# ElesionKyrie/Extreme-Video-Compression-With-Prediction-Using-Pre-trainded-Diffusion-Models-

Measured on AMD Instinct MI355X. Metric: decoded frames/sec (128x128x30) at q3, higher is better.
Workload: dtype f32

## Files before the change

extreme-video-compression-with-prediction-using-pre-trainded-diffusion-models-_amd/csrc/conv_igemm.hip:

```cpp
#include <hip/hip_runtime.h>
#include <stdint.h>
#include <stdio.h>
#include "../../include/evc_hip.h"

typedef float f32x16 __attribute__((ext_vector_type(16)));
typedef __attribute__((address_space(3))) void lds_void;
typedef const __attribute__((address_space(1))) void glb_void;

#ifndef EVC_CONV_TAIL
#define EVC_CONV_TAIL 1
#endif
#ifndef EVC_CONV_TM1
#define EVC_CONV_TM1 1
#endif
#ifndef EVC_SPLIT_WIDE_TILES
#define EVC_SPLIT_WIDE_TILES 1
#endif

#ifndef EVC_SPLIT_INTERLEAVE
#define EVC_SPLIT_INTERLEAVE 5
#endif

namespace {

// ... 1019 lines not shown
            __builtin_amdgcn_sched_barrier(0);
            asm volatile("s_waitcnt vmcnt(2) lgkmcnt(0)\n\ts_barrier" ::: "memory");
            __builtin_amdgcn_sched_barrier(0);
            wb ^= 1; ++sidx;
        }
        {
            EVC_RR_NEXT_W()
            EVC_RR_FRAGS(1)
            EVC_RR_TERMS(0, SP::NTERM)
            __syncthreads();
            wb ^= 1; ++sidx;
        }
        {
            EVC_RR_NEXT_W()
            __builtin_amdgcn_sched_barrier(0);
            EVC_RR_FRAGS(2)
            EVC_RR_TERMS(0, SP::NTERM / 2)
            __builtin_amdgcn_sched_barrier(0);
            store_a(ab ^ 1);
            __builtin_amdgcn_sched_barrier(0);
            EVC_RR_TERMS(SP::NTERM / 2, SP::NTERM)
            __builtin_amdgcn_sched_barrier(0);
            __syncthreads();
            wb ^= 1; ++sidx;
        }
    }
#undef EVC_RR_TERMS
#undef EVC_RR_FRAGS
#undef EVC_RR_NEXT_W

    conv_epilogue<TM, TN, WM>(p, acc, m0, n0, split, wm, wn, l31, half, tail);
}

template <bool PARTIAL, bool RES, bool STATS, bool ACT>
__device__ __forceinline__ void wide_epilogue_t(const ConvK& p, f32x16 (&acc)[4][3], char* lds, int m0, int n0, int split,
                                                int wave, int lane, bool tail) {
    constexpr int TM = 4, TN = 3, BM = 256, RS = 36;
    const int wm = wave >> 1, wn = wave & 1;
    const int l31 = lane & 31, half = lane >> 5;
    const int ws_m0 = tail ? p.tail_first * BM : 0;
    const size_t ws_M = tail ? (size_t)p.tail_rows : (size_t)p.M;
    const float ascale = p.w_hdr[0] / in_scale(p);
    const float oscale = p.out_scale;
    const bool has_res = RES && (!ACT || p.res != nullptr), has_stats = STATS && (!ACT || p.stats != nullptr);
    float* const patch0 = reinterpret_cast<float*>(lds) + wave * 2 * 32 * RS;
    const int wr = lane >> 3, wc = (lane & 7) * 4;
    const int mw = m0 + wm * 32 * TM;
    const int prow = 4 * half * RS + l31;
    constexpr int RD = 4;
    float4 rq[RD][4];
    const auto res_load = [&](int t, float4 (&dst)[4]) {
        const int jj = t / TM, ii = t - jj * TM;
        const float* rp = p.res + (size_t)(mw + ii * 32 + wr) * p.ld_res + n0 + wn * 32 * TN + jj * 32 + wc;
#pragma unroll
        for (int k = 0; k < 4; ++k) dst[k] = *reinterpret_cast<const float4*>(rp + (size_t)(8 * k) * p.ld_res);
    };
    if (has_res) {
#pragma unroll
        for (int t = 0; t < RD - 1; ++t) res_load(t, rq[t]);
    }
#pragma unroll
    for (int j = 0; j < TN; ++j) {
        const int cj = n0 + wn * 32 * TN + j * 32;
        const float bias = (!PARTIAL && p.bias) ? p.bias[cj + l31] : 0.f;
        float4 ssum = make_float4(0.f, 0.f, 0.f, 0.f), ssq = make_float4(0.f, 0.f, 0.f, 0.f);
#pragma unroll
        for (int i = 0; i < TM; ++i) {
            const int mb = mw + i * 32;
            const int tt = j * TM + i;
            if (has_res && tt + RD - 1 < TM * TN) res_load(tt + RD - 1, rq[(tt + RD - 1) % RD]);
            float* const P = patch0 + ((i * TN + j) & 1) * 32 * RS;
#pragma unroll
            for (int r = 0; r < 16; ++r) P[prow + ((r & 3) + 8 * (r >> 2)) * RS] = acc[i][j][r] * ascale + bias;
#pragma unroll
            for (int k = 0; k < 4; ++k) {
                float4 q = *reinterpret_cast<const float4*>(P + (wr + 8 * k) * RS + wc);
                const int m = mb + wr + 8 * k;
                if (!PARTIAL) {
                    if (has_res) { const float4& rr = rq[tt % RD][k]; q.x += rr.x; q.y += rr.y; q.z += rr.z; q.w += rr.w; }
                    q.x *= oscale; q.y *= oscale; q.z *= oscale; q.w *= oscale;
                    if (ACT) { q.x = act_fn(q.x, p.act_out); q.y = act_fn(q.y, p.act_out); q.z = act_fn(q.z, p.act_out); q.w = act_fn(q.w, p.act_out); }
                    if (STATS) {
                        ssum.x += q.x; ssum.y += q.y; ssum.z += q.z; ssum.w += q.w;
                        ssq.x += q.x * q.x; ssq.y += q.y * q.y; ssq.z += q.z * q.z; ssq.w += q.w * q.w;
                    }
                }
                float* dst = PARTIAL ? p.ws + ((size_t)split * ws_M + (m - ws_m0)) * p.Co + cj + wc
                                     : p.out + (size_t)m * p.ld_out + cj + wc;
                *reinterpret_cast<float4*>(dst) = q;
            }
            if (has_stats && (i & 1)) {
#pragma unroll
                for (int d = 8; d <= 32; d <<= 1) {
                    ssum.x += __shfl_xor(ssum.x, d); ssum.y += __shfl_xor(ssum.y, d); ssum.z += __shfl_xor(ssum.z, d); ssum.w += __shfl_xor(ssum.w, d);
                    ssq.x += __shfl_xor(ssq.x, d); ssq.y += __shfl_xor(ssq.y, d); ssq.z += __shfl_xor(ssq.z, d); ssq.w += __shfl_xor(ssq.w, d);
                }
                if (wr == 0) {
                    float* sp = p.stats + ((size_t)(m0 / 64 + wm * 2 + (i >> 1)) * p.Co + cj + wc) * 2;
                    *reinterpret_cast<float4*>(sp) = make_float4(ssum.x, ssq.x, ssum.y, ssq.y);
                    *reinterpret_cast<float4*>(sp + 4) = make_float4(ssum.z, ssq.z, ssum.w, ssq.w);
                }
                ssum = make_float4(0.f, 0.f, 0.f, 0.f); ssq = make_float4(0.f, 0.f, 0.f, 0.f);
            }
        }
    }
}

__device__ __forceinline__ void wide_epilogue(const ConvK& p, f32x16 (&acc)[4][3], char* lds, int m0, int n0, int split,
                                              int wave, int lane, bool tail) {
    const bool partial = p.splits > 1 || tail;
    if (partial) wide_epilogue_t<true, false, false, false>(p, acc, lds, m0, n0, split, wave, lane, tail);
    else if (p.act_out != EVC_ACT_NONE) wide_epilogue_t<false, true, true, true>(p, acc, lds, m0, n0, split, wave, lane, tail);
    else if (p.res && p.stats) wide_epilogue_t<false, true, true, false>(p, acc, lds, m0, n0, split, wave, lane, tail);
    else if (p.stats) wide_epilogue_t<false, false, true, false>(p, acc, lds, m0, n0, split, wave, lane, tail);
    else if (p.res) wide_epilogue_t<false, true, false, false>(p, acc, lds, m0, n0, split, wave, lane, tail);
    else wide_epilogue_t<false, false, false, false>(p, acc, lds, m0, n0, split, wave, lane, tail);
}

#ifndef EVC_WIDE_VMEM_EVERY
#define EVC_WIDE_VMEM_EVERY 36
#endif
#ifndef EVC_WIDE_BDIST
#define EVC_WIDE_BDIST 1
#endif
#ifndef EVC_WIDE_BUFFER_LOADS
#define EVC_WIDE_BUFFER_LOADS 0
#endif
#ifndef EVC_WIDE_ABL
#define EVC_WIDE_ABL 0
#endif
#ifdef EVC_WIDE_STAMPS
__device__ unsigned long long g_wide_stamps[8192 * 8];
#define EVC_STAMP(k) if (threadIdx.x == 0) g_wide_stamps[(blockIdx.x & 8191) * 8 + (k)] = __builtin_readcyclecounter();
#else
#define EVC_STAMP(k)
#endif
template <int MODE, int NU, bool X2>
__global__ __launch_bounds__(256, 1) void conv_wide_kernel(ConvK p) {
    typedef Split<2> SP;
    typedef f16x8 vec;
    constexpr int TM = 4, TN = 3, BM = 256, BN = 192, RB = 32;
    constexpr bool HAS_COEF = MODE == MODE_AFFINE || MODE == MODE_AFFINE_SILU;
    extern __shared__ __attribute__((aligned(16))) char smem_b[];
    const int W = p.W, SW = W + 2;
    const int R = BM / W;
    const int SPX = (R + 2) * SW;
    const int APL = SPX * RB;
    const int HPL = SPX * 16;
    char* const As = smem_b;

    const int tid = threadIdx.x;
    const int lane = tid & 63;
    const int wave = __builtin_amdgcn_readfirstlane(tid >> 6);
    const int wm = wave >> 1, wn = wave & 1;
    const int l31 = lane & 31, half = lane >> 5;

#ifdef EVC_WIDE_STAGGER_TEST
    if (blockIdx.x < 256) for (int q = 0; q < (int)((blockIdx.x >> 3) & 3) * EVC_WIDE_STAGGER_TEST; ++q) __builtin_amdgcn_s_sleep(127);
#endif
    EVC_STAMP(0)
    const bool tail = (int)blockIdx.x >= p.tail_first;
    const int tq = tail ? ((int)blockIdx.x - p.tail_first) / p.tail_splits : 0;
    const int m0 = (tail ? p.tail_first + tq : (int)blockIdx.x) * BM;
    const int n0 = blockIdx.y * BN;
    const int split = tail ? (int)blockIdx.x - p.tail_first - tq * p.tail_splits : (int)blockIdx.z;
    const int sps = tail ? p.tail_sps : p.steps_per_split;
    const int c_begin = p.cut_chunk ? (split ? p.cut_chunk : 0) : min(p.nchunk, split * (sps / 9));
    const int c_end = p.cut_chunk ? (split ? p.nchunk : p.cut_chunk) : min(p.nchunk, c_begin + sps / 9);

    const int bimg = m0 / p.HW;
    const int y0 = (m0 - bimg * p.HW) / W;
    const int Ct = p.C0 + p.C1;

    const int kh = tid & 1;
    unsigned goff0[NU], goff1[NU];
    int slds[NU];
    bool sval[NU], sex[NU];
#pragma unroll
    for (int k = 0; k < NU; ++k) {
        int pp = (tid + 256 * k) >> 1;
        if (pp >= (R + 2) * W) pp = tid >> 1;
        const int sr = pp / W, x = pp - sr * W;
        sex[k] = true;
        const int y = y0 + sr - 1;
        sval[k] = sex[k] && y >= 0 && y < p.H;
        const unsigned pix = (unsigned)((bimg * p.H + (sval[k] ? y : 0)) * W + x);
        goff0[k] = (pix * (unsigned)p.ld0 + 8u * kh) * 4u;
        goff1[k] = (pix * (unsigned)p.ld1 + 8u * kh) * 4u;
        const int spx = (sex[k] ? sr : 0) * SW + x + 1;
        slds[k] = kh * HPL + spx * 16;
    }
    int abase[TM];
#pragma unroll
    for (int i = 0; i < TM; ++i) {
        const int ml = wm * 128 + i * 32 + l31;
        const int r = ml / W, x = ml - r * W;
        abase[i] = half * HPL + (r * SW + x) * 16;
    }
    const auto tap_off = [&](int t) { return ((t / 3) * SW + (t % 3)) * 16; };
    const unsigned planeB = (unsigned)p.CoPad * RB;
    const unsigned slab = 2u * planeB;
    const unsigned w_tap = (unsigned)p.nchunk * slab;
    const unsigned wlane = (unsigned)(n0 + wn * 96 + l31) * RB + 16u * (unsigned)(half ^ ((l31 >> 3) & 1));
    const char* const wbase = reinterpret_cast<const char*>(p.w);
#if EVC_WIDE_BUFFER_LOADS
    typedef int i32x4 __attribute__((ext_vector_type(4)));
    const __amdgpu_buffer_rsrc_t wrsrc = __builtin_amdgcn_make_buffer_rsrc(const_cast<char*>(wbase), 0, 0x7fffffff, 0x00020000);
    auto load_b = [&](vec (&bb)[TN][2], int c, int t) {
        const int so = (int)((unsigned)t * w_tap + (unsigned)c * slab);
#pragma unroll
        for (int j = 0; j < TN; ++j) {
            const i32x4 q0 = __builtin_amdgcn_raw_buffer_load_b128(wrsrc, (int)wlane + j * 32 * RB, so, 0);
            const i32x4 q1 = __builtin_amdgcn_raw_buffer_load_b128(wrsrc, (int)(wlane + planeB) + j * 32 * RB, so, 0);
            bb[j][0] = __builtin_bit_cast(vec, q0);
            bb[j][1] = __builtin_bit_cast(vec, q1);
        }
    };
#else
    auto load_b = [&](vec (&bb)[TN][2], int c, int t) {
        const char* wt = wbase + ((unsigned)t * w_tap + (unsigned)c * slab);
#pragma unroll
        for (int j = 0; j < TN; ++j) {
            bb[j][0] = *reinterpret_cast<const vec*>(wt + wlane + j * 32 * RB);
            bb[j][1] = *reinterpret_cast<const vec*>(wt + planeB + wlane + j * 32 * RB);
        }
    };
#endif

    const float xscale = F16_ACT_SCALE * in_scale(p);
    float4 xr[NU][2], ca[2], cs[2];
// ... 16 lines not shown
        }
    };
    auto stage_store = [&](int k, int buf) {
        vec pl[2];
        SP::split(transform<MODE>(xr[k][0], ca[0], cs[0], sval[k]), transform<MODE>(xr[k][1], ca[1], cs[1], sval[k]), xscale, pl);
        char* A = As + buf * 2 * APL + slds[k];
        *reinterpret_cast<vec*>(A) = pl[0];
        *reinterpret_cast<vec*>(A + APL) = pl[1];
    };
    auto read_a = [&](int i, const char* img, int toff) {
        a[i][0] = *reinterpret_cast<const vec*>(img + abase[i] + toff);
        a[i][1] = *reinterpret_cast<const vec*>(img + APL + abase[i] + toff);
    };

    f32x16 acc[TM][TN];
#pragma unroll
    for (int i = 0; i < TM; ++i)
#pragma unroll
        for (int j = 0; j < TN; ++j)
#pragma unroll
            for (int r = 0; r < 16; ++r) acc[i][j][r] = 0.f;

    vec b[3][TN][2];
    const bool early = !X2 && c_begin < c_end;
    if (early) {
        coef_load(c_begin);
#pragma unroll
        for (int k = 0; k < NU; ++k) stage_load(k, c_begin);
        load_b(b[0], c_begin, 0);
    }
    EVC_STAMP(5)
    {
        const int nimg = X2 ? 3 : 2;
        const int per_img = (R + 2) * 2 * 4;
        for (int u = tid; u < nimg * per_img; u += 256) {
            const int img = u / per_img, q = u - img * per_img;
            const int ph = q & 3, side = (q >> 2) & 1, row = q >> 3;
            const int spx = row * SW + (side ? W + 1 : 0);
            *reinterpret_cast<float4*>(As + img * 2 * APL + (ph >> 1) * APL + (ph & 1) * HPL + spx * 16) = make_float4(0.f, 0.f, 0.f, 0.f);
        }
    }
    __syncthreads();

#define EVC_PIN(x) asm volatile("" : "+v"(x))
#define EVC_PIN4(f) asm volatile("" : "+v"((f).x), "+v"((f).y), "+v"((f).z), "+v"((f).w))
#define EVC_WIDE_MFMA_I(I, BB)                                                                          \
    _Pragma("unroll") for (int t_ = 0; t_ < SP::NTERM; ++t_)                                            \
        _Pragma("unroll") for (int j = 0; j < TN; ++j)                                                  \
            acc[I][j] = SP::mfma(a[I][SP::qa(t_)], BB[j][SP::qb(t_)], acc[I][j]);

    if constexpr (X2) {
        const int nch2 = (p.x2_C0 + p.x2_C1) / KC;
        const int nsp = tail ? p.tail_splits : p.splits;
        const int per = (nch2 + nsp - 1) / nsp;
        const int c2b = min(nch2, split * per), c2e = min(nch2, c2b + per);
        float s2 = 1.0f;
        {
            const float bb = sqrtf(__uint_as_float(*p.x2_bound));
            if (!(bb < 3.0e38f)) s2 = __builtin_nanf("");
            else if (bb > 0.f) s2 = ldexpf(1.0f, 6 - ilogbf(bb));
        }
        const float xscale2 = F16_ACT_SCALE * s2;
        const unsigned slab2 = 2u * planeB;
        float4 x2r[2][2][2];
        unsigned x2o0[2], x2o1[2];
        int x2l[2];
#pragma unroll
        for (int k = 0; k < 2; ++k) {
            const int pp = (tid + 256 * k) >> 1;
            const int r = pp / W, x = pp - r * W;
            x2o0[k] = ((unsigned)(m0 + pp) * (unsigned)p.x2_ld0 + 8u * kh) * 4u;
            x2o1[k] = ((unsigned)(m0 + pp) * (unsigned)p.x2_ld1 + 8u * kh) * 4u;
            x2l[k] = kh * HPL + ((r + 1) * SW + x + 1) * 16;
        }
        auto load2 = [&](int c, float4 (&xr2)[2][2]) {
            const int cc = c * KC;
            const bool first = cc < p.x2_C0;
            const char* src = reinterpret_cast<const char*>(first ? p.x2_src0 : p.x2_src1);
            const unsigned cb = (unsigned)(first ? cc : cc - p.x2_C0) * 4u;
#pragma unroll
            for (int k = 0; k < 2; ++k) {
                const unsigned o = (first ? x2o0[k] : x2o1[k]) + cb;
                xr2[k][0] = *reinterpret_cast<const float4*>(src + o);
                xr2[k][1] = *reinterpret_cast<const float4*>(src + o + 16);
            }
        };
        auto store2 = [&](int buf, float4 (&xr2)[2][2]) {
            const float4 z = make_float4(0.f, 0.f, 0.f, 0.f);
#pragma unroll
            for (int k = 0; k < 2; ++k) {
                vec pl[2];
                SP::split(transform<MODE_PLAIN>(xr2[k][0], z, z, true), transform<MODE_PLAIN>(xr2[k][1], z, z, true), xscale2, pl);
                char* A = As + buf * 2 * APL + x2l[k];
                *reinterpret_cast<vec*>(A) = pl[0];
                *reinterpret_cast<vec*>(A + APL) = pl[1];
            }
        };
        vec b2[2][TN][2];
        auto load_b2 = [&](vec (&bb)[TN][2], int c) {
            const char* wt = p.x2_w + (unsigned)c * slab2;
#pragma unroll
            for (int j = 0; j < TN; ++j) {
                bb[j][0] = *reinterpret_cast<const vec*>(wt + wlane + j * 32 * RB);
                bb[j][1] = *reinterpret_cast<const vec*>(wt + planeB + wlane + j * 32 * RB);
            }
        };
// ... 107 lines not shown
            __builtin_amdgcn_sched_group_barrier(0x200, 2, 0);                                          \
            __builtin_amdgcn_sched_barrier(0);                                                          \
            TAIL_CODE                                                                                   \
            __builtin_amdgcn_sched_barrier(0);                                                          \
        }
        EVC_WIDE_STEP(0, 0, -1, )
        EVC_WIDE_STEP(1, 1, -1, )
        EVC_WIDE_STEP(2, 2, 0, )
        EVC_WIDE_STEP(3, 3, 1, )
        EVC_WIDE_STEP(4, -1, 2, )
        EVC_WIDE_STEP(5, -1, 3, )
        EVC_WIDE_STEP(6, -1, -1, )
        EVC_WIDE_STEP(7, -1, -1, asm volatile("s_waitcnt lgkmcnt(0)\n\ts_barrier" ::: "memory");)
        EVC_WIDE_STEP(8, -1, -1, )
#undef EVC_WIDE_STEP
    }
#undef EVC_WIDE_MFMA_I
#undef EVC_PIN
#undef EVC_PIN4

    if (EVC_WIDE_ABL & 16) {
        float sacc = 0.f;
#pragma unroll
        for (int i = 0; i < TM; ++i)
#pragma unroll
            for (int j = 0; j < TN; ++j)
#pragma unroll
                for (int e = 0; e < 16; ++e) sacc += acc[i][j][e];
        p.out[(size_t)m0 * p.ld_out + tid] = sacc;
        return;
    }
    EVC_STAMP(2)
    __syncthreads();
    wide_epilogue(p, acc, As, (EVC_WIDE_ABL & 128) ? 0 : m0, n0, split, wave, lane, tail);
#ifdef EVC_WIDE_STAMPS
    asm volatile("s_waitcnt vmcnt(0)" ::: "memory");
    EVC_STAMP(3)
    if (threadIdx.x == 0) g_wide_stamps[(blockIdx.x & 8191) * 8 + 4] = __builtin_amdgcn_s_getreg(6 | (8 << 6) | (3 << 11)) ;
#endif
}

__global__ __launch_bounds__(1024) void conv_splitk_reduce_kernel(const float* __restrict__ ws, int splits, int M,
                                                                  int Co, const float* __restrict__ bias,
                                                                  const float* __restrict__ res, int ld_res,
                                                                  float scale, int act, float* __restrict__ out,
                                                                  int ld_out, float* __restrict__ stats) {
    __shared__ float red[2][16][64];
    const int l = threadIdx.x & 63;
    const int c = blockIdx.y * 64 + l;
    const int rg = threadIdx.x >> 6;
    const int m_base = blockIdx.x * 64;
    const size_t total = (size_t)M * Co;
    float s_sum = 0.f, s_sq = 0.f;
    if (c < Co) {
        const float b = bias ? bias[c] : 0.f;
        float v[4];
        size_t idx[4];
        bool ok[4];
#pragma unroll
        for (int k = 0; k < 4; ++k) {
            const int m = m_base + rg + 16 * k;
            ok[k] = m < M;
            idx[k] = (size_t)(ok[k] ? m : 0) * Co + c;
            v[k] = 0.f;
        }
        for (int z = 0; z < splits; ++z) {
            const float* w = ws + (size_t)z * total;
#pragma unroll
            for (int k = 0; k < 4; ++k) v[k] += w[idx[k]];
        }
#pragma unroll
        for (int k = 0; k < 4; ++k) {
            if (!ok[k]) continue;
// ... 145 lines not shown
    } else {
        if (hipMemsetAsync(packed, 0, F16_HDR_BYTES, st) != hipSuccess) return EVC_ELAUNCH;
        const size_t n = (size_t)Co * Ci * KH * KW;
        hipLaunchKernelGGL(conv_absmax_kernel, dim3(grid), dim3(256), 0, st, w, n, reinterpret_cast<unsigned*>(packed) + 2);
        hipLaunchKernelGGL(conv_pack_f16_kernel, dim3(grid), dim3(256), 0, st, w, (char*)packed, Co,
                           evc_conv_co_pad(Co), Ci, KH, KW);
    }
    return hipGetLastError() == hipSuccess ? EVC_OK : EVC_ELAUNCH;
}

static int conv_validate(const evc_conv_args* a) {
    if (!a || !a->src0 || !a->w_packed || !a->out) return EVC_EINVAL;
    if (a->C0 <= 0 || a->C0 % KC != 0 || a->C1 < 0 || a->C1 % KC != 0) return EVC_EINVAL;
    if (a->C1 > 0 && !a->src1) return EVC_EINVAL;
    if ((a->ld0 != 0 && (a->ld0 < a->C0 || (a->ld0 & 3))) || (a->ld1 != 0 && (a->ld1 < a->C1 || (a->ld1 & 3))))
        return EVC_EINVAL;
    if ((a->coef_a == nullptr) != (a->coef_s == nullptr)) return EVC_EINVAL;
    if (a->B <= 0 || a->H <= 0 || a->W <= 0 || a->Co <= 0) return EVC_EINVAL;
    if (a->KH <= 0 || a->KW <= 0 || !(a->KH & 1) || !(a->KW & 1)) return EVC_EINVAL;
    if (a->ld_out < a->Co || (a->res && a->ld_res < a->Co)) return EVC_EINVAL;
    if ((long long)a->B * a->H * a->W > 0x7fffffffLL) return EVC_EINVAL;
    if (a->arith != EVC_ARITH_F32 && a->arith != EVC_ARITH_BF16X6 && a->arith != EVC_ARITH_F16X3) return EVC_EINVAL;
    if (a->x2_w_packed) {
        if (!a->x2_src0 || !a->x2_bound || a->x2_C0 <= 0 || a->x2_C0 % KC != 0 || a->x2_C1 < 0 || a->x2_C1 % KC != 0) return EVC_EINVAL;
        if (a->x2_C1 > 0 && !a->x2_src1) return EVC_EINVAL;
        if ((a->x2_ld0 != 0 && (a->x2_ld0 < a->x2_C0 || (a->x2_ld0 & 3))) || (a->x2_ld1 != 0 && (a->x2_ld1 < a->x2_C1 || (a->x2_ld1 & 3))))
            return EVC_EINVAL;
    }
    return EVC_OK;
}

struct TileCfg { int tm, tn, bm, bn; long long tiles; int splits; int reuse; int wide; int steps_per_split;
                 int tail_first, tail_tiles, tail_splits, tail_sps;
                 int cut_chunk; };
static int g_wide_cut = 1;
static int g_tail_split = EVC_CONV_TAIL;
static int g_wide_tiles = EVC_SPLIT_WIDE_TILES;
static int g_no_reuse = 0;
static int g_wide_mid = 1;
static int g_wide256 = 1;
static int g_force_tm = 0;

static void split_tile_cfg(const evc_conv_args* a, long long M, long long ntile, int nsteps, TileCfg& c, bool rr_ok) {
    const double K = (double)a->KH * a->KW * (a->C0 + a->C1);
    const bool f16 = a->arith == EVC_ARITH_F16X3 && rr_ok;
    const double E = f16 ? 20.0 : 6.0, F2 = f16 ? 1.5 : 1.0;
    const auto grid_time = [&](long long n, double sps) {
        const long long R = n / 512, rem = n - R * 512;
        return (sps + E) * ((double)R * F2 + (rem == 0 ? 0.0 : (rem <= 256 && f16 ? 1.0 : F2)));
    };
    double best = 1e300;
    int best_tm = 2, best_s = 1;
    c.tail_first = 0; c.tail_tiles = 0; c.tail_splits = 1; c.tail_sps = 0;
    for (int tm = 2; tm >= 1; --tm) {
        if (g_force_tm && tm != g_force_tm) continue;
        const long long tiles = ((M + 64 * tm - 1) / (64 * tm)) * ntile;
        const int smax = a->splits > 0 ? a->splits : (nsteps / 4 < 1 ? 1 : (nsteps / 4 > 32 ? 32 : nsteps / 4));
        for (int s = a->splits > 0 ? a->splits : 1; s <= smax; ++s) {
            const double sps = (double)((nsteps + s - 1) / s);
            const double slab_mb = (double)s * (double)M * a->Co * 4.0 / 1e6;
            const double pen = s > 1 ? 1.0 + (slab_mb > 192.0 ? 300.0 : 40.0) * s / K : 1.0;
            const double tmf = tm == 1 ? (a->KH * a->KW > 1 ? 0.5 / (rr_ok ? 0.55 : 0.75) : 0.5) : 1.0;
            const double t = grid_time(tiles * s, sps) * pen * tmf;
            if (t < best * 0.9999) { best = t; best_tm = tm; best_s = s; }
        }
    }
    c.tm = best_tm;
    c.bm = 64 * c.tm;
    c.tiles = ((M + c.bm - 1) / c.bm) * ntile;
    c.splits = best_s;
    if (rr_ok && g_tail_split && a->splits <= 0 && !g_force_tm && M % 128 == 0) {
        const long long tm_all = M / 128, wgs = tm_all * ntile;
        const long long R = wgs / 512;
// ... 4 lines not shown
            if (ts > nsteps / unit) ts = nsteps / unit;
            if (ts >= 2) {
                int sps = (nsteps + ts - 1) / ts;
                sps = (sps + 2) / 3 * 3;
                ts = (nsteps + sps - 1) / sps;
                const double t_tail = grid_time(main_m * ntile, (double)nsteps) +
                                      grid_time(tail_m * ntile * ts, (double)sps) * (1.0 + 40.0 * ts / K);
                if (ts >= 2 && t_tail < best * 0.98) {
                    c.tm = 2; c.bm = 128; c.tiles = wgs; c.splits = 1;
                    c.tail_first = (int)main_m; c.tail_tiles = (int)tail_m; c.tail_splits = ts; c.tail_sps = sps;
                }
            }
        }
    }
}

static inline bool is_split_arith(int arith) { return arith == EVC_ARITH_BF16X6 || arith == EVC_ARITH_F16X3; }
static inline int arith_planes(int arith) { return arith == EVC_ARITH_F16X3 ? 2 : 3; }
constexpr long long LDS_CAP = 160 * 1024;

static long long rr_lds_bytes(int np, int bm, int W, int bn) {
    return (long long)np * 32 * (2LL * (bm / W) * (W + 2) + 2LL * bn);
}

static long long wide_lds_bytes(int W, bool x2) { return (x2 ? 6LL : 4LL) * (256 / W + 2) * (W + 2) * 32; }

static bool wide_ok(const evc_conv_args* a) {
    const bool mode_ok = a->coef_a ? a->act_in == EVC_ACT_SILU : a->act_in == EVC_ACT_NONE;
    return g_wide256 && mode_ok && a->arith == EVC_ARITH_F16X3 && a->KH == 3 && a->KW == 3 && a->Co % 192 == 0 &&
           (a->W == 16 || a->W == 32 || a->W == 64 || a->W == 128) && ((long long)a->H * a->W) % 256 == 0 &&
           a->ld_out % 4 == 0 && (!a->res || a->ld_res % 4 == 0);
}

static TileCfg conv_tile_cfg(const evc_conv_args* a) {
    TileCfg c;
    c.wide = 0;
    c.cut_chunk = 0;
    const long long M = (long long)a->B * a->H * a->W;
    const int CoPad = evc_conv_co_pad(a->Co);
    c.tn = pick_tn(CoPad);
    c.bn = 64 * c.tn;
    const long long ntile = CoPad / c.bn;
    const int nsteps = a->KH * a->KW * ((a->C0 + a->C1) / KC);
    c.reuse = 0;
    if (is_split_arith(a->arith)) {
        const int np = arith_planes(a->arith);
        const bool rr_ok = !g_no_reuse && a->KH == 3 && a->KW == 3 && a->W >= 4 && 128 % a->W == 0 &&
                           rr_lds_bytes(np, 128, a->W, c.bn) <= LDS_CAP;
        split_tile_cfg(a, M, ntile, nsteps, c, rr_ok);
        if (rr_ok && c.tm == 2) c.reuse = 1;
        if (c.reuse && c.splits == 1 && !c.tail_tiles && g_wide_tiles && M % 256 == 0 && rr_lds_bytes(np, 256, a->W, c.bn) <= LDS_CAP) {
            const long long t256 = (M / 256) * ntile;
            if ((t256 >= 512 && t256 % 256 == 0) || t256 >= 6 * 256) {
                c.bm = 256;
                c.tiles = t256;
            }
        }
    } else {
        c.tail_first = 0; c.tail_tiles = 0; c.tail_splits = 1; c.tail_sps = 0;
        c.tm = (!EVC_CONV_TM1 || ((M + 127) / 128) * ntile >= 64) ? 2 : 1;
        if (g_force_tm) c.tm = g_force_tm;
        c.bm = 64 * c.tm;
        c.tiles = ((M + c.bm - 1) / c.bm) * ntile;
        long long splits = 1;
        if (a->splits > 0) splits = a->splits;
        else if (c.tiles < 384) {
            splits = (640 + c.tiles / 2) / c.tiles;
            const int max_by_steps = nsteps / 8 > 0 ? nsteps / 8 : 1;
            if (splits > max_by_steps) splits = max_by_steps;
// ... 25 lines not shown
        if (g_wide_mid && wgs >= 32) {
            const int nchunk = (a->C0 + a->C1) / KC;
            int best_s = 0;
            double best_t = 1e300;
            for (int sp = 1; sp <= 8 && wgs * sp <= 256 && nchunk / sp >= 4; ++sp) {
                const int cps = (nchunk + sp - 1) / sp;
                const double slab_mb = sp > 1 ? (double)sp * M * a->Co * 4.0 / 1e6 : 0.0;
                const double t = 23000.0 + 13900.0 * cps + (sp > 1 ? 2.0 * 2000.0 * (5.0 + slab_mb / 4.0) : 0.0);
                if (t < best_t) { best_t = t; best_s = sp; }
            }
            if (best_s > 0 && wgs * best_s >= 128) {
                const int cps = (nchunk + best_s - 1) / best_s;
                c.wide = 1; c.reuse = 0; c.tm = 4; c.tn = 3; c.bm = 256; c.bn = 192; c.tiles = wgs;
                c.tail_first = 0; c.tail_tiles = 0; c.tail_splits = 1; c.tail_sps = 0;
                c.splits = (nchunk + cps - 1) / cps;
                c.steps_per_split = cps * 9;
                if (g_wide_cut && best_s == 1 && wgs > 128 && nchunk >= 6) {
                    const long long idle = 256 - wgs, r = (wgs + idle - 1) / idle;
                    const double slab_mb = 2.0 * M * a->Co * 4.0 / 1e6;
                    const double comb = 2.0 * 2000.0 * (5.0 + slab_mb / 4.0);
                    int cut = 0;
                    double t_cut = best_t * 0.95;
                    for (int sh = 1; sh <= nchunk / 2; ++sh) {
                        const double tl = 23000.0 + 13900.0 * (nchunk - sh), ts = (double)r * (23000.0 + 13900.0 * sh);
                        const double t = (tl > ts ? tl : ts) + comb;
                        if (t < t_cut) { t_cut = t; cut = nchunk - sh; }
                    }
                    if (cut > 0) { c.splits = 2; c.cut_chunk = cut; c.steps_per_split = cut * 9; }
                }
                return c;
            }
        }
    }
    const int unit = c.reuse ? a->KW : 1;
    int sps = (nsteps + c.splits - 1) / c.splits;
    sps = (sps + unit - 1) / unit * unit;
    c.steps_per_split = sps;
    c.splits = (nsteps + sps - 1) / sps;
    return c;
}

extern "C" int evc_conv_set_option(const char* name, int value) {
    if (!name) return EVC_EINVAL;
    const auto is = [&](const char* s) { int i = 0; while (s[i] && s[i] == name[i]) ++i; return s[i] == 0 && name[i] == 0; };
    if (is("wide_tiles")) { g_wide_tiles = value; return EVC_OK; }
    if (is("row_reuse")) { g_no_reuse = !value; return EVC_OK; }
    if (is("tail_split")) { g_tail_split = value; return EVC_OK; }
    if (is("wide256")) { g_wide256 = value; return EVC_OK; }
    if (is("wide_mid")) { g_wide_mid = value; return EVC_OK; }
    if (is("wide_cut")) { g_wide_cut = value; return EVC_OK; }
    return EVC_EINVAL;
}

extern "C" int evc_conv_fused_1x1_supported(const evc_conv_args* a) {
    if (conv_validate(a) != EVC_OK) return 0;
    if (a->arith != EVC_ARITH_F16X3 || a->KH != 3 || a->KW != 3) return 0;
    const TileCfg c = conv_tile_cfg(a);
    return (c.reuse == 1 || c.wide) ? 1 : 0;
}

extern "C" int evc_conv_kernel_name(const evc_conv_args* a, char* buf, int n) {
    if (!buf || n <= 0 || conv_validate(a) != EVC_OK) return EVC_EINVAL;
    int mode;
    if (a->coef_a) mode = a->act_in == EVC_ACT_SILU ? MODE_AFFINE_SILU : MODE_AFFINE;
    else mode = a->act_in == EVC_ACT_SILU ? MODE_SILU : a->act_in == EVC_ACT_RELU ? MODE_RELU : MODE_PLAIN;
    const TileCfg c = conv_tile_cfg(a);
    int len;
    if (c.wide) len = snprintf(buf, n, "conv_wide_kernel<%d, %d, %s>", mode, a->W == 128 ? 4 : 3, a->x2_w_packed ? "true" : "false");
    else if (is_split_arith(a->arith)) {
        const int np = arith_planes(a->arith);
        if (c.reuse) len = snprintf(buf, n, "conv_split_rr_kernel<%d, %d, %d, %d>", np, c.bm == 256 ? 4 : 2, c.tn, mode);
        else if (np == 3) len = snprintf(buf, n, "conv_split_kernel<%d, %d, %d>", c.tm, c.tn, mode);
        else len = snprintf(buf, n, "conv_splitn_kernel<2, %d, %d, %d>", c.tm, c.tn, mode);
    } else len = snprintf(buf, n, "conv_igemm_kernel<%d, %d, %d>", c.tm, c.tn, mode);
    return len;
}

extern "C" int evc_conv_choose_splits(const evc_conv_args* a) {
    if (conv_validate(a) != EVC_OK) return EVC_EINVAL;
    return conv_tile_cfg(a).splits;
}

extern "C" int evc_conv_stats_splits(const evc_conv_args* a) {
    if (conv_validate(a) != EVC_OK) return 0;
    const int HW = a->H * a->W;
    if (HW % 64 != 0) return 0;
    const TileCfg c = conv_tile_cfg(a);
    if (c.splits > 1 || c.wide) return HW / 64;
    const long long M = (long long)a->B * HW;
    const int CoPad = evc_conv_co_pad(a->Co);
    if (M % c.bm != 0 || a->Co != CoPad || a->Co % c.bn != 0) return 0;
    return HW / (32 * c.tm);
}

extern "C" long long evc_conv_workspace_bytes(const evc_conv_args* a) {
    if (conv_validate(a) != EVC_OK) return EVC_EINVAL;
    const TileCfg c = conv_tile_cfg(a);
    if (c.tail_tiles) return (long long)c.tail_splits * c.tail_tiles * c.bm * a->Co * (long long)sizeof(float);
    if (c.splits == 1) return 0;
    return (long long)c.splits * a->B * a->H * a->W * a->Co * (long long)sizeof(float);
}
// ... 53 lines not shown
    const int rc = ensure_dynamic_lds(reinterpret_cast<const void*>(&conv_split_rr_kernel<NP, WM, TN, MODE>), &attr_done, lds);
    if (rc != EVC_OK) return rc;
    hipLaunchKernelGGL((conv_split_rr_kernel<NP, WM, TN, MODE>), grid, dim3(128 * WM), lds, st, k);
    return EVC_OK;
}
template <int NP, int WM, int TN>
static int launch_split_rr(int mode, dim3 grid, size_t lds, hipStream_t st, const ConvK& k) {
    int rc = EVC_OK;
#define EVC_CALL(M) rc = launch_split_rr_one<NP, WM, TN, M>(grid, lds, st, k)
    EVC_MODE_SWITCH(mode, EVC_CALL)
#undef EVC_CALL
    return rc;
}

template <int MODE, int NU, bool X2>
static int launch_wide_one(dim3 grid, size_t lds, hipStream_t st, const ConvK& k) {
    static unsigned long long attr_done = 0;
    const int rc = ensure_dynamic_lds(reinterpret_cast<const void*>(&conv_wide_kernel<MODE, NU, X2>), &attr_done, lds);
    if (rc != EVC_OK) return rc;
    hipLaunchKernelGGL((conv_wide_kernel<MODE, NU, X2>), grid, dim3(256), lds, st, k);
    return EVC_OK;
}
template <int MODE>
static int launch_wide_mode(int nu, bool x2, dim3 grid, size_t lds, hipStream_t st, const ConvK& k) {
    if (nu == 4) return x2 ? launch_wide_one<MODE, 4, true>(grid, lds, st, k) : launch_wide_one<MODE, 4, false>(grid, lds, st, k);
    return x2 ? launch_wide_one<MODE, 3, true>(grid, lds, st, k) : launch_wide_one<MODE, 3, false>(grid, lds, st, k);
}
static int launch_wide(int mode, int nu, bool x2, dim3 grid, size_t lds, hipStream_t st, const ConvK& k) {
#ifdef EVC_DEV_FAST
    return launch_wide_mode<MODE_AFFINE_SILU>(nu, x2, grid, lds, st, k);
#else
    if (mode == MODE_AFFINE_SILU) return launch_wide_mode<MODE_AFFINE_SILU>(nu, x2, grid, lds, st, k);
    if (mode == MODE_PLAIN) return launch_wide_mode<MODE_PLAIN>(nu, x2, grid, lds, st, k);
    return EVC_EUNSUPPORTED;
#endif
}

#define EVC_TN_SWITCH(tn, CALL) ((tn) == 3 ? CALL(3) : (tn) == 2 ? CALL(2) : CALL(1))

static int conv2d_impl(const evc_conv_args* a, float* ws, void* stream, hipEvent_t ev_start, hipEvent_t ev_conv_end);

extern "C" int evc_conv2d_nhwc_f32(const evc_conv_args* a, float* ws, void* stream) {
    return conv2d_impl(a, ws, stream, nullptr, nullptr);
}

extern "C" int evc_conv2d_nhwc_profiled_f32(const evc_conv_args* a, float* ws, void* stream, void* ev_start,
                                            void* ev_conv_end) {
    return conv2d_impl(a, ws, stream, (hipEvent_t)ev_start, (hipEvent_t)ev_conv_end);
}

static int conv2d_impl(const evc_conv_args* a, float* ws, void* stream, hipEvent_t ev_start, hipEvent_t ev_conv_end) {
    int rc = conv_validate(a);
    if (rc != EVC_OK) return rc;
    int mode;
    if (a->coef_a) {
        if (a->act_in == EVC_ACT_SILU) mode = MODE_AFFINE_SILU;
        else if (a->act_in == EVC_ACT_NONE) mode = MODE_AFFINE;
        else return EVC_EUNSUPPORTED;
    } else {
        mode = a->act_in == EVC_ACT_SILU ? MODE_SILU : a->act_in == EVC_ACT_RELU ? MODE_RELU : MODE_PLAIN;
        if (a->act_in != EVC_ACT_NONE && a->act_in != EVC_ACT_SILU && a->act_in != EVC_ACT_RELU) return EVC_EINVAL;
    }
    ConvK k;
    k.src0 = a->src0; k.src1 = a->src1 ? a->src1 : a->src0; k.C0 = a->C0; k.C1 = a->C1;
    k.ld0 = a->ld0 > 0 ? a->ld0 : a->C0; k.ld1 = a->ld1 > 0 ? a->ld1 : (a->C1 > 0 ? a->C1 : k.ld0);
    k.coef_a = a->coef_a; k.coef_s = a->coef_s;
// ... 17 lines not shown
    k.nchunk = (a->C0 + a->C1) / KC;
    k.nsteps = a->KH * a->KW * k.nchunk;
    const TileCfg cfg = conv_tile_cfg(a);
    k.splits = cfg.splits;
    k.steps_per_split = cfg.steps_per_split;
    k.ws = ws;
    if ((k.splits > 1 || cfg.tail_tiles) && !ws) return EVC_EINVAL;
    k.stats = k.splits > 1 ? nullptr : a->stats_out;
    if (a->stats_out && evc_conv_stats_splits(a) == 0) return EVC_EINVAL;
    k.x2_w = nullptr; k.x2_hdr = nullptr; k.x2_bound = nullptr; k.x2_src0 = k.x2_src1 = nullptr;
    k.x2_C0 = k.x2_C1 = k.x2_ld0 = k.x2_ld1 = 0;
    if (a->x2_w_packed) {
        if (a->arith != EVC_ARITH_F16X3 || a->KH != 3 || a->KW != 3 || !(cfg.reuse == 1 || cfg.wide)) return EVC_EUNSUPPORTED;
        k.x2_src0 = a->x2_src0; k.x2_src1 = a->x2_src1 ? a->x2_src1 : a->x2_src0;
        k.x2_C0 = a->x2_C0; k.x2_C1 = a->x2_C1;
        k.x2_ld0 = a->x2_ld0 > 0 ? a->x2_ld0 : a->x2_C0;
        k.x2_ld1 = a->x2_ld1 > 0 ? a->x2_ld1 : (a->x2_C1 > 0 ? a->x2_C1 : k.x2_ld0);
        if ((long long)k.M * k.x2_ld0 * 4 >= (1LL << 32) || (long long)k.M * k.x2_ld1 * 4 >= (1LL << 32)) return EVC_EUNSUPPORTED;
        k.x2_hdr = a->x2_w_packed;
        k.x2_w = reinterpret_cast<const char*>(a->x2_w_packed) + F16_HDR_BYTES;
        k.x2_bound = a->x2_bound;
    }
    k.tail_first = 0x7fffffff; k.tail_splits = 1; k.tail_sps = 0; k.tail_rows = 0;
    k.cut_chunk = cfg.wide ? cfg.cut_chunk : 0;
    if (cfg.tail_tiles) {
        k.tail_first = cfg.tail_first; k.tail_splits = cfg.tail_splits; k.tail_sps = cfg.tail_sps;
        k.tail_rows = cfg.tail_tiles * cfg.bm;
    }

    dim3 grid((k.M + cfg.bm - 1) / cfg.bm, k.CoPad / cfg.bn, k.splits);
    if (cfg.tail_tiles) grid.x = cfg.tail_first + cfg.tail_tiles * cfg.tail_splits;
    hipStream_t st = (hipStream_t)stream;
    if (ev_start && hipEventRecord(ev_start, st) != hipSuccess) return EVC_ELAUNCH;
    if (cfg.wide) {
        rc = launch_wide(mode, a->W == 128 ? 4 : 3, a->x2_w_packed != nullptr, grid, (size_t)wide_lds_bytes(a->W, a->x2_w_packed != nullptr), st, k);
    } else if (is_split_arith(a->arith)) {
        const int np = arith_planes(a->arith);
        if (cfg.reuse) {
            const size_t lds_rr = (size_t)rr_lds_bytes(np, cfg.bm, a->W, cfg.bn);
#define EVC_RR4_3(TN) launch_split_rr<3, 4, TN>(mode, grid, lds_rr, st, k)
#define EVC_RR2_3(TN) launch_split_rr<3, 2, TN>(mode, grid, lds_rr, st, k)
#define EVC_RR4_2(TN) launch_split_rr<2, 4, TN>(mode, grid, lds_rr, st, k)
#define EVC_RR2_2(TN) launch_split_rr<2, 2, TN>(mode, grid, lds_rr, st, k)
            if (np == 3) rc = cfg.bm == 256 ? EVC_TN_SWITCH(cfg.tn, EVC_RR4_3) : EVC_TN_SWITCH(cfg.tn, EVC_RR2_3);
            else rc = cfg.bm == 256 ? EVC_TN_SWITCH(cfg.tn, EVC_RR4_2) : EVC_TN_SWITCH(cfg.tn, EVC_RR2_2);
#undef EVC_RR4_3
#undef EVC_RR2_3
#undef EVC_RR4_2
#undef EVC_RR2_2
        } else {
            const size_t lds = (size_t)2 * np * (cfg.bm + cfg.bn) * 32;
#define EVC_S3_2(TN) launch_split3<2, TN>(mode, grid, lds, st, k)
#define EVC_S3_1(TN) launch_split3<1, TN>(mode, grid, lds, st, k)
#define EVC_S2_2(TN) launch_split2<2, TN>(mode, grid, lds, st, k)
#define EVC_S2_1(TN) launch_split2<1, TN>(mode, grid, lds, st, k)
            if (np == 3) rc = cfg.tm == 2 ? EVC_TN_SWITCH(cfg.tn, EVC_S3_2) : EVC_TN_SWITCH(cfg.tn, EVC_S3_1);
            else rc = cfg.tm == 2 ? EVC_TN_SWITCH(cfg.tn, EVC_S2_2) : EVC_TN_SWITCH(cfg.tn, EVC_S2_1);
#undef EVC_S3_2
#undef EVC_S3_1
#undef EVC_S2_2
#undef EVC_S2_1
        }
    } else {
        const size_t lds = (size_t)2 * (cfg.bm + cfg.bn) * KC * sizeof(float);
#define EVC_F_2(TN) launch_mode<2, TN>(mode, grid, lds, st, k)
#define EVC_F_1(TN) launch_mode<1, TN>(mode, grid, lds, st, k)
        rc = cfg.tm == 2 ? EVC_TN_SWITCH(cfg.tn, EVC_F_2) : EVC_TN_SWITCH(cfg.tn, EVC_F_1);
// ... 23 lines not shown
```

Measured before the change: 35.11.

## Add small-spatial wide conv kernel packing multiple images per tile with split-K

Adds a SMALL variant of the wide implicit-GEMM conv kernel for 8x8 and 16x16 feature maps. Each 256-row tile packs several whole images with their own halo rows in LDS, and partial results are written masked to a split-K workspace. A cost model picks the chunks per split so that small low-resolution layers fill more of the GPU instead of falling back to the reuse kernel. The trade-off is extra split-K reduction traffic and halo overhead per image.

```diff
diff --git a/extreme-video-compression-with-prediction-using-pre-trainded-diffusion-models-_amd/csrc/conv_igemm.hip b/extreme-video-compression-with-prediction-using-pre-trainded-diffusion-models-_amd/csrc/conv_igemm.hip
--- a/extreme-video-compression-with-prediction-using-pre-trainded-diffusion-models-_amd/csrc/conv_igemm.hip
+++ b/extreme-video-compression-with-prediction-using-pre-trainded-diffusion-models-_amd/csrc/conv_igemm.hip
@@ -1075,7 +1075,7 @@
     conv_epilogue<TM, TN, WM>(p, acc, m0, n0, split, wm, wn, l31, half, tail);
 }
 
-template <bool PARTIAL, bool RES, bool STATS, bool ACT>
+template <bool PARTIAL, bool RES, bool STATS, bool ACT, bool MASK = false>
 __device__ __forceinline__ void wide_epilogue_t(const ConvK& p, f32x16 (&acc)[4][3], char* lds, int m0, int n0, int split,
                                                 int wave, int lane, bool tail) {
     constexpr int TM = 4, TN = 3, BM = 256, RS = 36;
@@ -1130,7 +1130,7 @@
                 }
                 float* dst = PARTIAL ? p.ws + ((size_t)split * ws_M + (m - ws_m0)) * p.Co + cj + wc
                                      : p.out + (size_t)m * p.ld_out + cj + wc;
-                *reinterpret_cast<float4*>(dst) = q;
+                if (!MASK || m < p.M) *reinterpret_cast<float4*>(dst) = q;
             }
             if (has_stats && (i & 1)) {
 #pragma unroll
@@ -1178,8 +1178,8 @@
 #else
 #define EVC_STAMP(k)
 #endif
-template <int MODE, int NU, bool X2>
-__global__ __launch_bounds__(256, 1) void conv_wide_kernel(ConvK p) {
+template <int MODE, int NU, bool X2, bool SMALL>
+__device__ __forceinline__ void conv_wide_body(const ConvK& p) {
     typedef Split<2> SP;
     typedef f16x8 vec;
     constexpr int TM = 4, TN = 3, BM = 256, BN = 192, RB = 32;
@@ -1187,7 +1187,8 @@
     extern __shared__ __attribute__((aligned(16))) char smem_b[];
     const int W = p.W, SW = W + 2;
     const int R = BM / W;
-    const int SPX = (R + 2) * SW;
+    const int SR = SMALL ? (BM / p.HW) * (p.H + 2) : R + 2;
+    const int SPX = SR * SW;
     const int APL = SPX * RB;
     const int HPL = SPX * 16;
     char* const As = smem_b;
@@ -1211,8 +1212,12 @@
     const int c_begin = p.cut_chunk ? (split ? p.cut_chunk : 0) : min(p.nchunk, split * (sps / 9));
     const int c_end = p.cut_chunk ? (split ? p.nchunk : p.cut_chunk) : min(p.nchunk, c_begin + sps / 9);
 
-    const int bimg = m0 / p.HW;
-    const int y0 = (m0 - bimg * p.HW) / W;
+    const int TPI = SMALL ? 256 / (BM / p.HW) : 256;
+    const int img_t = SMALL ? tid / TPI : 0;
+    const int bimg_u = m0 / p.HW + img_t;
+    const bool bval = !SMALL || bimg_u < p.B;
+    const int bimg = SMALL ? min(bimg_u, p.B - 1) : bimg_u;
+    const int y0 = SMALL ? 0 : (m0 - bimg * p.HW) / W;
     const int Ct = p.C0 + p.C1;
 
     const int kh = tid & 1;
@@ -1221,16 +1226,17 @@
     bool sval[NU], sex[NU];
 #pragma unroll
     for (int k = 0; k < NU; ++k) {
-        int pp = (tid + 256 * k) >> 1;
-        if (pp >= (R + 2) * W) pp = tid >> 1;
+        const int tu = SMALL ? tid % TPI : tid;
+        int pp = (tu + TPI * k) >> 1;
+        if (pp >= (SMALL ? p.H + 2 : R + 2) * W) pp = tu >> 1;
         const int sr = pp / W, x = pp - sr * W;
         sex[k] = true;
         const int y = y0 + sr - 1;
-        sval[k] = sex[k] && y >= 0 && y < p.H;
+        sval[k] = sex[k] && bval && y >= 0 && y < p.H;
         const unsigned pix = (unsigned)((bimg * p.H + (sval[k] ? y : 0)) * W + x);
         goff0[k] = (pix * (unsigned)p.ld0 + 8u * kh) * 4u;
         goff1[k] = (pix * (unsigned)p.ld1 + 8u * kh) * 4u;
-        const int spx = (sex[k] ? sr : 0) * SW + x + 1;
+        const int spx = ((sex[k] ? sr : 0) + img_t * (p.H + 2)) * SW + x + 1;
         slds[k] = kh * HPL + spx * 16;
     }
     int abase[TM];
@@ -1238,7 +1244,8 @@
     for (int i = 0; i < TM; ++i) {
         const int ml = wm * 128 + i * 32 + l31;
         const int r = ml / W, x = ml - r * W;
-        abase[i] = half * HPL + (r * SW + x) * 16;
+        const int sr = SMALL ? r + 2 * (r / p.H) : r;
+        abase[i] = half * HPL + (sr * SW + x) * 16;
     }
     const auto tap_off = [&](int t) { return ((t / 3) * SW + (t % 3)) * 16; };
     const unsigned planeB = (unsigned)p.CoPad * RB;
@@ -1321,7 +1328,7 @@
     EVC_STAMP(5)
     {
         const int nimg = X2 ? 3 : 2;
-        const int per_img = (R + 2) * 2 * 4;
+        const int per_img = SR * 2 * 4;
         for (int u = tid; u < nimg * per_img; u += 256) {
             const int img = u / per_img, q = u - img * per_img;
             const int ph = q & 3, side = (q >> 2) & 1, row = q >> 3;
@@ -1358,9 +1365,11 @@
         for (int k = 0; k < 2; ++k) {
             const int pp = (tid + 256 * k) >> 1;
             const int r = pp / W, x = pp - r * W;
-            x2o0[k] = ((unsigned)(m0 + pp) * (unsigned)p.x2_ld0 + 8u * kh) * 4u;
-            x2o1[k] = ((unsigned)(m0 + pp) * (unsigned)p.x2_ld1 + 8u * kh) * 4u;
-            x2l[k] = kh * HPL + ((r + 1) * SW + x + 1) * 16;
+            const int sr = SMALL ? r + 2 * (r / p.H) : r;
+            const unsigned m = (unsigned)(SMALL ? min(m0 + pp, p.M - 1) : m0 + pp);
+            x2o0[k] = (m * (unsigned)p.x2_ld0 + 8u * kh) * 4u;
+            x2o1[k] = (m * (unsigned)p.x2_ld1 + 8u * kh) * 4u;
+            x2l[k] = kh * HPL + ((sr + 1) * SW + x + 1) * 16;
         }
         auto load2 = [&](int c, float4 (&xr2)[2][2]) {
             const int cc = c * KC;
@@ -1534,13 +1543,20 @@
     }
     EVC_STAMP(2)
     __syncthreads();
-    wide_epilogue(p, acc, As, (EVC_WIDE_ABL & 128) ? 0 : m0, n0, split, wave, lane, tail);
+    if constexpr (SMALL) wide_epilogue_t<true, false, false, false, true>(p, acc, As, m0, n0, split, wave, lane, false);
+    else wide_epilogue(p, acc, As, (EVC_WIDE_ABL & 128) ? 0 : m0, n0, split, wave, lane, tail);
 #ifdef EVC_WIDE_STAMPS
     asm volatile("s_waitcnt vmcnt(0)" ::: "memory");
     EVC_STAMP(3)
     if (threadIdx.x == 0) g_wide_stamps[(blockIdx.x & 8191) * 8 + 4] = __builtin_amdgcn_s_getreg(6 | (8 << 6) | (3 << 11)) ;
 #endif
 }
+
+template <int MODE, int NU, bool X2>
+__global__ __launch_bounds__(256, 1) void conv_wide_kernel(ConvK p) { conv_wide_body<MODE, NU, X2, false>(p); }
+
+template <int MODE, bool X2>
+__global__ __launch_bounds__(256, 1) void conv_small_kernel(ConvK p) { conv_wide_body<MODE, 3, X2, true>(p); }
 
 __global__ __launch_bounds__(1024) void conv_splitk_reduce_kernel(const float* __restrict__ ws, int splits, int M,
                                                                   int Co, const float* __restrict__ bias,
@@ -1752,13 +1768,15 @@
 
 struct TileCfg { int tm, tn, bm, bn; long long tiles; int splits; int reuse; int wide; int steps_per_split;
                  int tail_first, tail_tiles, tail_splits, tail_sps;
-                 int cut_chunk; };
+                 int cut_chunk;
+                 int small; };
 static int g_wide_cut = 1;
 static int g_tail_split = EVC_CONV_TAIL;
 static int g_wide_tiles = EVC_SPLIT_WIDE_TILES;
 static int g_no_reuse = 0;
 static int g_wide_mid = 1;
 static int g_wide256 = 1;
+static int g_small_grid = 1;
 static int g_force_tm = 0;
 
 static void split_tile_cfg(const evc_conv_args* a, long long M, long long ntile, int nsteps, TileCfg& c, bool rr_ok) {
@@ -1829,9 +1847,19 @@
            a->ld_out % 4 == 0 && (!a->res || a->ld_res % 4 == 0);
 }
 
+static bool small_ok(const evc_conv_args* a) {
+    const bool mode_ok = a->coef_a ? a->act_in == EVC_ACT_SILU : a->act_in == EVC_ACT_NONE;
+    const int HW = a->H * a->W;
+    return g_small_grid && mode_ok && a->arith == EVC_ARITH_F16X3 && a->KH == 3 && a->KW == 3 && a->Co % 192 == 0 &&
+           (a->W == 8 || a->W == 16) && HW <= 256 && 256 % HW == 0 && a->ld_out % 4 == 0 && (!a->res || a->ld_res % 4 == 0);
+}
+
+static long long small_lds_bytes(int H, int W, bool x2) { return (x2 ? 6LL : 4LL) * (256 / (H * W)) * (H + 2) * (W + 2) * 32; }
+
 static TileCfg conv_tile_cfg(const evc_conv_args* a) {
     TileCfg c;
     c.wide = 0;
+    c.small = 0;
     c.cut_chunk = 0;
     const long long M = (long long)a->B * a->H * a->W;
     const int CoPad = evc_conv_co_pad(a->Co);
@@ -1923,6 +1951,30 @@
             }
         }
     }
+    if (c.reuse && small_ok(a) && a->splits <= 0 && !g_force_tm) {
+        const long long tiles = (M + 255) / 256, nt = a->Co / 192, wgs = tiles * nt;
+        const int nchunk = (a->C0 + a->C1) / KC;
+        const int nch2 = a->x2_w_packed ? (a->x2_C0 + a->x2_C1) / KC : 0;
+        int best_cps = 0;
+        double best_t = 1e300;
+        const bool pays = nchunk >= 36 && (nch2 == 0 || a->W == 16 || a->Co >= 768);
+        if (pays && 2 * M >= tiles * 256) {
+            for (int sp = 2; sp <= nchunk; ++sp) {
+                const int cps = (nchunk + sp - 1) / sp, s_eff = (nchunk + cps - 1) / cps;
+                if (s_eff < 2 || wgs * s_eff > 256) continue;
+                const double slab_mb = (double)s_eff * M * a->Co * 4.0 / 1e6;
+                const double t = (23000.0 + 13900.0 * cps + 3000.0 * ((nch2 + s_eff - 1) / s_eff)) / 2100.0 + 5.0 + 0.2 * slab_mb;
+                if (t < best_t) { best_t = t; best_cps = cps; }
+            }
+        }
+        if (best_cps > 0) {
+            c.wide = 1; c.small = 1; c.reuse = 0; c.tm = 4; c.tn = 3; c.bm = 256; c.bn = 192; c.tiles = wgs;
+            c.tail_first = 0; c.tail_tiles = 0; c.tail_splits = 1; c.tail_sps = 0;
+            c.splits = (nchunk + best_cps - 1) / best_cps;
+            c.steps_per_split = best_cps * 9;
+            return c;
+        }
+    }
     const int unit = c.reuse ? a->KW : 1;
     int sps = (nsteps + c.splits - 1) / c.splits;
     sps = (sps + unit - 1) / unit * unit;
@@ -1940,6 +1992,7 @@
     if (is("wide256")) { g_wide256 = value; return EVC_OK; }
     if (is("wide_mid")) { g_wide_mid = value; return EVC_OK; }
     if (is("wide_cut")) { g_wide_cut = value; return EVC_OK; }
+    if (is("small_grid")) { g_small_grid = value; return EVC_OK; }
     return EVC_EINVAL;
 }
 
@@ -1957,7 +2010,8 @@
     else mode = a->act_in == EVC_ACT_SILU ? MODE_SILU : a->act_in == EVC_ACT_RELU ? MODE_RELU : MODE_PLAIN;
     const TileCfg c = conv_tile_cfg(a);
     int len;
-    if (c.wide) len = snprintf(buf, n, "conv_wide_kernel<%d, %d, %s>", mode, a->W == 128 ? 4 : 3, a->x2_w_packed ? "true" : "false");
+    if (c.small) len = snprintf(buf, n, "conv_small_kernel<%d, %s>", mode, a->x2_w_packed ? "true" : "false");
+    else if (c.wide) len = snprintf(buf, n, "conv_wide_kernel<%d, %d, %s>", mode, a->W == 128 ? 4 : 3, a->x2_w_packed ? "true" : "false");
     else if (is_split_arith(a->arith)) {
         const int np = arith_planes(a->arith);
         if (c.reuse) len = snprintf(buf, n, "conv_split_rr_kernel<%d, %d, %d, %d>", np, c.bm == 256 ? 4 : 2, c.tn, mode);
@@ -2077,6 +2131,24 @@
 #else
     if (mode == MODE_AFFINE_SILU) return launch_wide_mode<MODE_AFFINE_SILU>(nu, x2, grid, lds, st, k);
     if (mode == MODE_PLAIN) return launch_wide_mode<MODE_PLAIN>(nu, x2, grid, lds, st, k);
+    return EVC_EUNSUPPORTED;
+#endif
+}
+
+template <int MODE, bool X2>
+static int launch_small_one(dim3 grid, size_t lds, hipStream_t st, const ConvK& k) {
+    static unsigned long long attr_done = 0;
+    const int rc = ensure_dynamic_lds(reinterpret_cast<const void*>(&conv_small_kernel<MODE, X2>), &attr_done, lds);
+    if (rc != EVC_OK) return rc;
+    hipLaunchKernelGGL((conv_small_kernel<MODE, X2>), grid, dim3(256), lds, st, k);
+    return EVC_OK;
+}
+static int launch_small(int mode, bool x2, dim3 grid, size_t lds, hipStream_t st, const ConvK& k) {
+#ifdef EVC_DEV_FAST
+    return x2 ? launch_small_one<MODE_AFFINE_SILU, true>(grid, lds, st, k) : launch_small_one<MODE_AFFINE_SILU, false>(grid, lds, st, k);
+#else
+    if (mode == MODE_AFFINE_SILU) return x2 ? launch_small_one<MODE_AFFINE_SILU, true>(grid, lds, st, k) : launch_small_one<MODE_AFFINE_SILU, false>(grid, lds, st, k);
+    if (mode == MODE_PLAIN) return x2 ? launch_small_one<MODE_PLAIN, true>(grid, lds, st, k) : launch_small_one<MODE_PLAIN, false>(grid, lds, st, k);
     return EVC_EUNSUPPORTED;
 #endif
 }
@@ -2160,7 +2232,9 @@
     if (cfg.tail_tiles) grid.x = cfg.tail_first + cfg.tail_tiles * cfg.tail_splits;
     hipStream_t st = (hipStream_t)stream;
     if (ev_start && hipEventRecord(ev_start, st) != hipSuccess) return EVC_ELAUNCH;
-    if (cfg.wide) {
+    if (cfg.small) {
+        rc = launch_small(mode, a->x2_w_packed != nullptr, grid, (size_t)small_lds_bytes(a->H, a->W, a->x2_w_packed != nullptr), st, k);
+    } else if (cfg.wide) {
         rc = launch_wide(mode, a->W == 128 ? 4 : 3, a->x2_w_packed != nullptr, grid, (size_t)wide_lds_bytes(a->W, a->x2_w_packed != nullptr), st, k);
     } else if (is_split_arith(a->arith)) {
         const int np = arith_planes(a->arith);
```

Measured after the change: 35.33 (median of 6 runs). About the same (+0.7%).
